# SamShue/EKF_SLAM

Hardware: AMD Instinct MI355X
Metric: EKF update-steps/sec at N landmarks; HBM GB/s on (I−KH)P vs roofline (higher is better)
Workload: dtype f64

## Files before the change

ekf_slam_amd/_lib.py:

```python
import ctypes
import os
import subprocess

_HERE = os.path.dirname(os.path.abspath(__file__))
LIB_PATH = os.environ.get("EKF_LIB_PATH") or os.path.join(_HERE, "libekfslam.so")

EKF_OK = 0
EKF_ERR_INVALID_ARG, EKF_ERR_NO_DEVICE, EKF_ERR_HIP, EKF_ERR_CAPACITY = 1, 2, 3, 4
EKF_ERR_INDEX, EKF_ERR_LOOKUP, EKF_ERR_STATE, EKF_ERR_COMM = 5, 6, 7, 8
EKF_MODE_KNOWN, EKF_MODE_UC = 0, 1
EKF_COMM_ID_BYTES = 128
EKF_MERGE_BATCH_MAX = 32
EKF_STORE_F64, EKF_STORE_F32 = 0, 1
EKF_ARITH_F64, EKF_ARITH_F32, EKF_ARITH_SPLIT3 = 0, 1, 2
(EKF_KERNEL_DOWNDATE, EKF_KERNEL_GATHER, EKF_KERNEL_PREDICT, EKF_KERNEL_ASSOCIATE, EKF_KERNEL_APPEND,
 EKF_KERNEL_ROWPANEL, EKF_KERNEL_EXCHANGE, EKF_KERNEL_COMPACT, EKF_KERNEL_COUNT) = range(9)

_d = ctypes.c_double
_dp = ctypes.POINTER(ctypes.c_double)
_i32 = ctypes.c_int32
_i64 = ctypes.c_int64
_vp = ctypes.c_void_p


class EkfConfig(ctypes.Structure):
    _fields_ = [("C", _d), ("Rc", _d * 2), ("s_cost", _d), ("s_thresh", _d), ("w_pos", _d),
                ("capacity_landmarks", _i64), ("mode", _i32), ("storage", _i32), ("device", _i32),
                ("tile", _i32), ("rank", _i32), ("world", _i32), ("batch", _i32), ("async_flush", _i32), ("device_assoc", _i32),
                ("pass_direction", _i32), ("force_sharded", _i32), ("pass_arith", _i32), ("reserved", _i32 * 2)]


class EkfLinearObs(ctypes.Structure):
    _fields_ = [("z", _d * 2), ("R", _d * 4), ("Hr", _d * 6), ("lm", _i64 * 2), ("Hl", (_d * 4) * 2), ("gate", _d),
                ("wrap_deg", _i32 * 2), ("rows", _i32)]


class EkfLinearResult(ctypes.Structure):
    _fields_ = [("nu", _d * 2), ("S", _d * 4), ("d2", _d), ("outcome", _i32)]


EKF_LINEAR_IRREGULAR, EKF_LINEAR_APPLIED, EKF_LINEAR_GATED = 0, 1, 2


class EkfModelObs(ctypes.Structure):
    _fields_ = [("model", _i32), ("reserved", _i32), ("z", _d * 2), ("R", _d * 4), ("lm", _i64 * 2), ("anchor", _d * 2), ("gate", _d)]


EKF_MODEL_RANGE_BEARING, EKF_MODEL_RANGE, EKF_MODEL_BEARING, EKF_MODEL_RELATIVE_XY, EKF_MODEL_LANDMARK_RANGE = 1, 2, 3, 4, 5
EKF_MODEL_ROWS = {1: 2, 2: 1, 3: 1, 4: 2, 5: 1}

EKF_APPEND_MODEL_MAX = 32

# ... 120 lines not shown
```

ekf_slam_amd/csrc/abi.hip:

```cpp
#include "host/handle.h"
#include "host/invalidate.h"
#include "host/exchange.h"
#include "host/passes.h"
#include "host/steps.h"
#include "host/assoc.h"
#include "host/measure.h"
#include "host/edits.h"
#include "host/linear.h"
#include "host/model.h"
#include "host/append_model.h"
#include "host/associate_model.h"
#include "host/state.h"
#include "host/lifecycle.h"

extern "C" {
int32_t ekf_abi_version(void) { return EKF_ABI_VERSION; }

const char *ekf_status_string(int32_t s) {
    switch (s) {
        case EKF_OK: return "ok";
        case EKF_ERR_INVALID_ARG: return "invalid argument";
        case EKF_ERR_NO_DEVICE: return "no HIP device";
        case EKF_ERR_HIP: return "HIP runtime error";
        case EKF_ERR_CAPACITY: return "landmark capacity exhausted";
// ... 35 lines not shown
    HIPCHK(h, hipStreamSynchronize(h->stream));
    h->stream = hip_stream ? (hipStream_t)hip_stream : h->own_stream;
    return EKF_OK;
}

int32_t ekf_sync(ekf_handle *h) {
    if (!h) return EKF_ERR_INVALID_ARG;
    TRY(enter(h));
    HIPCHK(h, hipStreamSynchronize(h->stream));
    if (h->flush_stream) HIPCHK(h, hipStreamSynchronize(h->flush_stream));
    return EKF_OK;
}

int32_t ekf_flush(ekf_handle *h) {
    if (!h) return EKF_ERR_INVALID_ARG;
    REQUIRE(h, !h->pending, EKF_ERR_STATE, "flush: a sharded correction is between begin and finish");
    int32_t rc = use_device(h);
    if (!rc) rc = settle(h);
    return rc ? rc : flush_pending(h);
}

int32_t ekf_pending(ekf_handle *h, int32_t *npending) {
    if (!h || !npending) return EKF_ERR_INVALID_ARG;
    *npending = h->npend;
    return EKF_OK;
}

int32_t ekf_set_params(ekf_handle *h, double C, const double Rc[2], double s_cost, double s_thresh, double w_pos) {
    if (!h || !Rc) return fail(h, EKF_ERR_INVALID_ARG, "set_params: null argument");
    h->cfg.C = C; h->cfg.Rc[0] = Rc[0]; h->cfg.Rc[1] = Rc[1];
    h->cfg.s_cost = s_cost; h->cfg.s_thresh = s_thresh; h->cfg.w_pos = w_pos;
    return EKF_OK;
}

int32_t ekf_predict(ekf_handle *h, const double u[2]) {
    if (!h || !u) return fail(h, EKF_ERR_INVALID_ARG, "predict: null argument");
    int32_t rc = use_device(h);
    return rc ? rc : do_predict(h, u);
}

int32_t ekf_motion_model(const double *x, int64_t n, const double u[2], double *x_new, double *F) {
    if (!x || !u || !x_new || n < 3) return EKF_ERR_INVALID_ARG;
    const double th = x[2];
    for (int64_t i = 0; i < n; ++i) x_new[i] = x[i];
    x_new[0] = x[0] + u[0] * ekfm::cosd(th + u[1]);
    x_new[1] = x[1] + u[0] * ekfm::sind(th + u[1]);
    x_new[2] = th + u[1];
    if (F) {
        for (int64_t i = 0; i < n * n; ++i) F[i] = 0.0;
        for (int64_t i = 0; i < n; ++i) F[i * n + i] = 1.0;
        F[2 * n + 0] = -1 * u[0] * ekfm::sind(th);
        F[2 * n + 1] = u[0] * ekfm::cosd(th);
    }
    return EKF_OK;
}

int32_t ekf_append(ekf_handle *h, const double u[2], const double R[4], const double pos[2], double signature) {
    if (!h || !u || !R || !pos) return fail(h, EKF_ERR_INVALID_ARG, "append: null argument");
    int32_t rc = use_device(h);
    if (!rc) rc = settle(h);
    return rc ? rc : do_append(h, u, R, pos, signature);
}

int32_t ekf_correct(ekf_handle *h, const double z[2], const double R[4], int64_t idx) {
    if (!h || !z || !R) return fail(h, EKF_ERR_INVALID_ARG, "correct: null argument");
    int32_t rc = use_device(h);
    if (!rc) rc = settle(h);
    return rc ? rc : do_correct(h, z, R, idx);
}

int32_t ekf_associate(ekf_handle *h, const double z[3], const double R[4], int32_t *is_new, int64_t *idx,
                      double *pos_cost, double *sig_cost) {
    if (!h || !z || !R || !is_new || !idx) return fail(h, EKF_ERR_INVALID_ARG, "associate: null argument");
    int32_t rc = use_device(h);
    if (!rc) rc = settle(h);
    return rc ? rc : do_associate(h, z, R, is_new, idx, pos_cost, sig_cost);
}

int32_t ekf_hint_next(ekf_handle *h, int64_t idx) {
    if (!h) return EKF_ERR_INVALID_ARG;
    h->hint_idx = (idx >= 0 && idx < h->N) ? idx : -1;
    return EKF_OK;
}

int32_t ekf_num_landmarks(ekf_handle *h, int64_t *N) {
    if (!h || !N) return fail(h, EKF_ERR_INVALID_ARG, "num_landmarks: null argument");
    if (unsettled(h) > 0) TRY(settle(h));
    *N = h->N;
    return EKF_OK;
}

// ... 21 lines not shown
```

ekf_slam_amd/csrc/host/handle.h:

```cpp
#pragma once
#include "../../../include/ekfslam.h"
#include <hip/hip_runtime.h>
#include <dlfcn.h>
#include <cstdio>
#include <cstdlib>
#include <algorithm>
#include <cmath>
#include <cstring>
#include <new>
#include <string>
#include <vector>

#include "../device_math.h"
#include "../flush32_pipe.h"
#include "../kernels.h"
#include "../layout.h"

struct KernelTimer {
    bool enabled = false;
    std::vector<hipEvent_t> ev;
    size_t used = 0;
};

struct ekf_handle {
    ekf_config cfg;
    int64_t N = 0;
    int64_t cap = 0;
    int32_t T = 64;
    int32_t storage = 0;
    int32_t cur = 0;
    DevState st;
    hipStream_t own_stream = nullptr, stream = nullptr;
    double *h_small = nullptr;
    double *d_digest = nullptr;
    bool have_pp = false;
    PredictArgs pp;
    std::vector<double> s_host;
    mutable std::vector<std::pair<double, int64_t>> s_sorted, s_tail;
    mutable bool s_sorted_ok = false;
    static constexpr size_t kSortedTail = 2048;
    hipEvent_t throttle_ev[2] = { nullptr, nullptr };
    bool throttle_set[2] = { false, false };
    int throttle_k = 0, since_mark = 0;
    int32_t batch = 1;
    int32_t npend = 0;
    int32_t pstart = 0;
    bool async_flush = false;
    void *tilebuf[2] = { nullptr, nullptr };
    int32_t base = 0;
    int32_t nfrozen = 0;
    bool inflight = false;
    int64_t inflight_N = 0;
    bool appended_inflight = false;
    const int64_t *inflight_dn = nullptr;
    int flush_cus = 0;
    hipStream_t flush_stream = nullptr;
    hipEvent_t ev_pairs = nullptr, ev_flushed = nullptr, ev_rows = nullptr;
    PassAux aux = { nullptr, 0, nullptr, 0, 0, nullptr, nullptr };
    int grid_cap = 0;
// ... 143 lines not shown
}

struct DevTemp {
    void **p;
    template <typename Tp> explicit DevTemp(Tp **q) : p((void **)q) {}
    ~DevTemp() { if (*p) hipFree(*p); }
};

template <typename Tp>
int32_t stage_alloc(ekf_handle *h, Tp **area, size_t bytes, hipEvent_t *ev) {
    if (!*area) HIPCHK(h, halloc(h, area, bytes ? bytes : 16, hipHostMallocDefault));
    if (!*ev) HIPCHK(h, new_event(h, ev));
    return EKF_OK;
}
int32_t stage_wait(ekf_handle *h, hipEvent_t ev, bool &busy) { if (busy) { HIPCHK(h, hipEventSynchronize(ev)); busy = false; } return EKF_OK; }
int32_t stage_uploaded(ekf_handle *h, hipEvent_t ev, bool &busy) { HIPCHK(h, hipEventRecord(ev, h->stream)); busy = true; return EKF_OK; }

inline int64_t n_mm(const ekf_handle *h) { return 2 * h->N; }
inline bool decided_mode(const ekf_handle *h) { return h->cfg.mode == EKF_MODE_UC && h->cfg.device_assoc == 4; }
inline int64_t unsettled(const ekf_handle *h) { return decided_mode(h) ? (int64_t)(h->lrec_head - h->lrec_tail) : 0; }
inline int64_t n_hi(const ekf_handle *h) { return h->N + unsettled(h); }
inline size_t elt_size(const ekf_handle *h) { return h->storage == EKF_STORE_F64 ? 8 : 4; }

int32_t use_device(ekf_handle *h) {
    HIPCHK(h, hipSetDevice(h->cfg.device));
    return EKF_OK;
}

struct TimedLaunch {
    hipStream_t s;
    KernelTimer *t;
    hipEvent_t stop = nullptr;
    TimedLaunch(ekf_handle *h, int which) : TimedLaunch(h, which, h->stream) {}
    TimedLaunch(ekf_handle *h, int which, hipStream_t on) : s(on), t(&h->timers[which]) {
        if (!t->enabled) { t = nullptr; return; }
        if (t->used + 2 > t->ev.size()) {
            hipEvent_t a, b;
            if (hipEventCreate(&a) != hipSuccess || hipEventCreate(&b) != hipSuccess) { t = nullptr; return; }
            t->ev.push_back(a); t->ev.push_back(b);
        }
        hipEventRecord(t->ev[t->used], s);
        stop = t->ev[t->used + 1];
        t->used += 2;
    }
    ~TimedLaunch() { if (t) hipEventRecord(stop, s); }
};

#define TIMED(h, which, call) do { TimedLaunch tl_((h), (which)); HIPCHK((h), call); } while (0)

// ... 5 lines not shown
```

ekf_slam_amd/csrc/host/lifecycle.h:

```cpp
#pragma once
namespace {
int32_t create_state(ekf_handle *h) {
    const int64_t ldm = h->st.ldm;
    for (int b = 0; b < 2; ++b) {
        HIPCHK(h, dalloc(h, &h->st.x[b], (size_t)(3 + ldm)));
        HIPCHK(h, dalloc(h, &h->st.prr[b], 16));
        HIPCHK(h, dalloc(h, &h->st.strip[b], (size_t)(3 * ldm)));
        HIPCHK(h, dalloc(h, &h->st.diag[b], (size_t)(3 * h->cap)));
    }
    h->st.dcur = 0;
    HIPCHK(h, dalloc(h, &h->st.s, (size_t)h->cap));
    HIPCHK(h, dalloc(h, &h->st.small, 32));
    HIPCHK(h, dalloc(h, &h->d_digest, kDigestDoubles));
    HIPCHK(h, dalloc(h, &h->d_csmall, 16));
    HIPCHK(h, halloc(h, &h->h_small, 32 * sizeof(double), hipHostMallocDefault));
    const double prr0[9] = { 0.1, 0, 0, 0, 0.1, 0, 0, 0, 0.1 };
    HIPCHK(h, hipMemcpy(h->st.prr[0], prr0, sizeof prr0, hipMemcpyHostToDevice));
    h->cur = 0;
    h->N = 0;
    return EKF_OK;
}
}

extern "C" {
int32_t ekf_create(const ekf_config *cfg, ekf_handle **out) {
    if (!cfg || !out) return EKF_ERR_INVALID_ARG;
    *out = nullptr;
    const int32_t T = cfg->tile == 0 ? (cfg->storage == EKF_STORE_F32 ? 256 : 128) : cfg->tile;
    const int32_t world = cfg->world <= 0 ? 1 : cfg->world;
    if (!(T == 16 || T == 32 || T == 64 || T == 128 || (T == 256 && cfg->storage == EKF_STORE_F32))) return EKF_ERR_INVALID_ARG;
    if (cfg->capacity_landmarks < 1 || cfg->rank < 0 || cfg->rank >= world) return EKF_ERR_INVALID_ARG;
    if (cfg->storage != EKF_STORE_F64 && cfg->storage != EKF_STORE_F32) return EKF_ERR_INVALID_ARG;
    if (cfg->mode != EKF_MODE_KNOWN && cfg->mode != EKF_MODE_UC) return EKF_ERR_INVALID_ARG;
    if (cfg->batch < 0 || cfg->batch > 64) return EKF_ERR_INVALID_ARG;
    if (cfg->mode == EKF_MODE_UC && cfg->device_assoc == 4 && (world > 1 || cfg->force_sharded)) return EKF_ERR_INVALID_ARG;
    if (cfg->pass_arith != EKF_ARITH_F64 &&
        !((cfg->pass_arith == EKF_ARITH_F32 || cfg->pass_arith == EKF_ARITH_SPLIT3) && cfg->storage == EKF_STORE_F32 && T == 256))
        return EKF_ERR_INVALID_ARG;
    int ndev = 0;
    if (hipGetDeviceCount(&ndev) != hipSuccess || ndev <= 0 || cfg->device < 0 || cfg->device >= ndev)
        return EKF_ERR_NO_DEVICE;

    ekf_handle *h = new (std::nothrow) ekf_handle();
    if (!h) return EKF_ERR_INVALID_ARG;
    h->cfg = *cfg;
    h->cfg.world = world;
    h->cfg.tile = T;
    h->T = T;
    h->cap = cfg->capacity_landmarks;
    h->storage = cfg->storage;
    *out = h;

    HIPCHK(h, hipSetDevice(cfg->device));
    hipDeviceProp_t prop = {};
    if (cfg->async_flush != 0 || cfg->pass_arith != EKF_ARITH_F64) HIPCHK(h, hipGetDeviceProperties(&prop, cfg->device));
    {
        int lo = 0, hi = 0;
        HIPCHK(h, hipDeviceGetStreamPriorityRange(&lo, &hi));
        HIPCHK(h, hipStreamCreateWithPriority(&h->own_stream, hipStreamNonBlocking, hi));
    }
    h->stream = h->own_stream;
    const int64_t nt_cap = ekf_tiles_for(2 * h->cap, T);
    h->st.ldm = nt_cap * T;
    h->st.tm = ekf_make_tilemap(T, world, cfg->rank);
    h->work_cap = h->st.tm.slots_for_rows(nt_cap);

    TRY(create_state(h));
    TRY(create_passes(h, prop));
    TRY(create_worklists(h));
    TRY(create_assoc(h));
    TRY(create_exchange(h));
    TRY(create_decided(h));
    TRY(create_linear(h));
// ... 58 lines not shown
```

ekf_slam_amd/csrc/host/steps.h:

```cpp
#pragma once
namespace {
int32_t verify_loop(ekf_handle *h, bool block);
void note_append(ekf_handle *h, double signature);

int32_t materialize_predict(ekf_handle *h) {
    if (!h->have_pp) return EKF_OK;
    h->have_pp = false;
    PredictArgs a = h->pp;
    a.n_mm = 2 * n_hi(h); a.cur = h->cur;
    TIMED(h, EKF_KERNEL_PREDICT, launch_predict(h->st, a, h->storage, h->stream));
    h->cur ^= 1;
    return EKF_OK;
}

int32_t do_predict(ekf_handle *h, const double u[2]) {
    TRY(materialize_predict(h));
    h->pp.u0 = u[0]; h->pp.u1 = u[1]; h->pp.C = h->cfg.C; h->pp.n_mm = 0; h->pp.cur = 0;
    h->have_pp = true;
    static const bool lazy = ekf_tune_int("EKF_LAZY_PREDICT", 1) != 0;
    return lazy ? EKF_OK : materialize_predict(h);
}

int32_t enter(ekf_handle *h) {
    HIPCHK(h, hipSetDevice(h->cfg.device));
    const int32_t rc = verify_loop(h,  true);
    return rc ? rc : materialize_predict(h);
}

int32_t enter_flushed(ekf_handle *h) { TRY(enter(h)); return flush_pending(h); }

int32_t do_append(ekf_handle *h, const double u[2], const double R[4], const double pos[2], double signature,
                  const DevLoopArgs *dl = nullptr) {
    REQUIRE(h, h->N < h->cap, EKF_ERR_CAPACITY, "append: capacity_landmarks exhausted");
    if (h->inflight) h->appended_inflight = true;
    AppendArgs a;
    a.u0 = u[0]; a.u1 = u[1];
    colmajor2(R, a.R00, a.R01, a.R10, a.R11);
    a.pos0 = pos[0]; a.pos1 = pos[1]; a.signature = signature; a.N = h->N; a.cur = h->cur;
    {
// ... 115 lines not shown
            return rc ? rc : finish_step(h);
        }
        int32_t rc = correct_begin(h, z, R, idx);
        if (!rc) rc = run_exchange(h);
        return rc ? rc : correct_finish(h);
    }
    TRY(refresh_work(h));
    CorrectArgs a;
    fill_correct_args(h, a, z, R, idx);
    static const bool fuse_small = ekf_tune_int("EKF_FUSE_SMALL", 1) != 0;
    const bool fused = fuse_small && h->batch == 1 && !h->async_flush && h->npend == 0 && a.n_mm <= gather_fuse_max_rows() &&
                       ekf_tiles_for(a.n_mm, h->T) * h->T <= 256;
    const PredictArgs *fuse = h->have_pp ? &h->pp : nullptr;
    TIMED(h, EKF_KERNEL_GATHER, launch_gather(h->st, a, fuse, h->storage, h->stream, fused));
    h->have_pp = false;
    if (fused) {
        h->cur ^= 1;
        h->st.dcur ^= 1;
        snprintf(h->dd_kernel, sizeof h->dd_kernel, "k_gather<%s,fused downdate>", h->storage == EKF_STORE_F64 ? "double" : "float");
        h->dd_pairs = 1;
        return throttle_step(h);
    }
    return finish_step(h);
}

int32_t do_correct_dev(ekf_handle *h, const double z[2], const double R[4], int64_t idx, const DevLoopArgs &dl) {
    REQUIRE(h, idx >= 0 && idx < h->N, EKF_ERR_INDEX, "correct: landmark index outside the state");
    TRY(refresh_work(h));
    CorrectArgs a;
    fill_correct_args(h, a, z, R, idx);
    if (h->sharded) {
        REQUIRE(h, !h->pending, EKF_ERR_STATE, "correct: an exchange is pending");
        h->slab = slab_for(h, a.n_mm);
        TIMED(h, EKF_KERNEL_ROWPANEL, launch_rowpanel_dev(h->st, a.j, a.n_mm, h->pstart, h->npend, corr_send(h, h->slab), h->storage, h->stream, dl));
        exchange_changed(h);
        h->x_count = h->slab;
        TRY(exchange_bracket(h, 1));
        TRY(gather_sharded(h, a, h->recv, h->slab, 0,  true, &dl));
        return finish_step(h);
    }
    const PredictArgs *fuse = h->have_pp ? &h->pp : nullptr;
    TIMED(h, EKF_KERNEL_GATHER, launch_gather_devloop(h->st, a, fuse, dl, h->storage, h->stream));
    h->have_pp = false;
    return finish_step(h);
}
}
// ... 56 lines not shown
```

ekf_slam_amd/csrc/kernel_args.h:

```cpp
#pragma once
#include <stdint.h>

#include "layout.h"

struct DevState {
    double *x[2];
    double *prr[2];
    double *strip[2];
    void   *tiles;
    double *s;
    double *Gp;
    double *Kp;
    float  *Gp32;
    float  *Kp32;
    int64_t pair_stride;
    int32_t pcap;
    double *small;
    int64_t ldm;
    TileMap tm;
    double *diag[2];
    int32_t dcur;
};

struct PredictArgs {
    double u0, u1, C;
    int64_t n_mm;
// ... 122 lines not shown
```

ekf_slam_amd/csrc/kernels.h:

```cpp
#pragma once
#include <hip/hip_runtime.h>
#include <stdint.h>

#include "device_math.h"
#include "kernel_args.h"
#include "layout.h"

#ifdef EKF_TUNING
#include <stdlib.h>
inline int ekf_tune_int(const char *name, int dflt) { const char *v = getenv(name); return v ? atoi(v) : dflt; }
#else
constexpr int ekf_tune_int(const char *, int dflt) { return dflt; }
#endif

hipError_t launch_predict(const DevState &st, const PredictArgs &a, int storage, hipStream_t s);

hipError_t launch_append(const DevState &st, const AppendArgs &a, int storage, hipStream_t s, const DevLoopArgs *dl = nullptr,
                         const PredictArgs *fused_predict = nullptr);

hipError_t launch_append_model(const DevState &st, const AppendModelArgs &a, int storage, hipStream_t s);

hipError_t launch_gather(const DevState &st, const CorrectArgs &a, const PredictArgs *fused_predict, int storage,
                         hipStream_t s, bool fuse_downdate);
int gather_fuse_max_rows();
hipError_t launch_gather_devloop(const DevState &st, const CorrectArgs &a, const PredictArgs *fused_predict, const DevLoopArgs &dl,
                                 int storage, hipStream_t s);
int64_t gather_workgroups(const DevState &st, int64_t n_mm);
hipError_t launch_gather_decided(const DevState &st, const CorrectArgs &a, const DevLoopArgs &dl, int storage, hipStream_t s);

hipError_t launch_rowpanel(const DevState &st, int64_t j, int64_t n_mm, int pstart, int npend, double *send, int storage,
                           hipStream_t s);
hipError_t launch_rowpanel_dev(const DevState &st, int64_t j, int64_t n_mm, int pstart, int npend, double *send, int storage,
                               hipStream_t s, const DevLoopArgs &dl);
struct RowList { int32_t m; int32_t j[64]; };
hipError_t launch_rowpanel_base(const DevState &st, const int64_t *idx, int m, int64_t n_mm, double *send, int64_t slab,
                                int storage, hipStream_t s);
hipError_t launch_rowpanel_next(const DevState &st, const int64_t *idx, int m, int64_t n_mm, int pstart, int npend, double *send,
                                int64_t slab, int storage, hipStream_t s);
hipError_t launch_gather_sharded(const DevState &st, const CorrectArgs &a, const PredictArgs *fused_predict, const double *recv,
                                 int64_t rank_stride, int64_t offset, bool patched, int storage, hipStream_t s,
                                 const DevLoopArgs *dl = nullptr);

struct AssocDecision {
    int64_t index;
    int32_t is_new;
    int32_t seq;
    double  min_ll;
// ... 84 lines not shown
```

ekf_slam_amd/csrc/kernels.hip:

```cpp
#include "kernels.h"

#include <algorithm>
#include <atomic>
#include <cstdio>
#include <type_traits>

#include "device_math.h"
#include "flush32_mfma.h"
#include "flush32_pipe.h"
#include "flush32_split.h"
#include "flush64_mfma.h"

namespace {

#include "tile_access.h"
#include "lane_ops.h"
#include "predict.h"
#include "assoc_winners.h"
#include "append.h"
#include "append_model.h"
#include "solve_small.h"
#include "rowpanel.h"
#include "pair_column.h"
#include "gather.h"
#include "downdate.h"
#include "associate.h"
#include "state_io.h"
#include "compact.h"
#include "constrain.h"
#include "linear_obs.h"
#include "model_obs.h"
#include "associate_model.h"
#include "merge_pass.h"
#include "nearest.h"

}

#include "launch/dispatch.h"
#include "launch/steps.h"
#include "launch/pass_select.h"
#include "launch/passes.h"
#include "launch/edits.h"
#include "launch/state_io.h"
```

ekf_slam_amd/csrc/launch/steps.h:

```cpp
#pragma once

hipError_t launch_predict(const DevState &st, const PredictArgs &a, int, hipStream_t s) {
    static const int force = ekf_tune_int("EKF_PREDICT_MFMA", -1);
    const bool mfma = force >= 0 ? force != 0 : a.n_mm >= 2048;
    if (mfma) {
        const int64_t nslices = (a.n_mm + 15) / 16;
        int64_t grid = cdiv(nslices > 0 ? nslices : 1, 4);
        if (grid > 1024) grid = 1024;
        hipLaunchKernelGGL(k_predict_mfma, dim3((unsigned)grid), dim3(kBlock), 0, s, st, a);
        return hipGetLastError();
    }
    const int64_t grid = cdiv(a.n_mm > 0 ? a.n_mm : 1, kBlock);
    hipLaunchKernelGGL(k_predict, dim3((unsigned)grid), dim3(kBlock), 0, s, st, a);
    return hipGetLastError();
}

hipError_t launch_append(const DevState &st, const AppendArgs &a, int storage, hipStream_t s, const DevLoopArgs *dlp,
                         const PredictArgs *fused_predict) {
    const int64_t n_mm = 2 * a.N;
    const int64_t grid = cdiv(n_mm > 0 ? n_mm : 1, kBlock);
    const DevLoopArgs dl = dlp ? *dlp : DevLoopArgs{};
    const PredictArgs pa = predict_or_none(fused_predict);
    return with_storage(storage, [&](auto ts) { with_bool(fused_predict != nullptr, [&](auto pred) {
        hipLaunchKernelGGL((k_append<decltype(ts), decltype(pred)::value>), dim3((unsigned)grid), dim3(kBlock), 0, s, st, a, dl, pa);
// ... 19 lines not shown
    typename DevLoopParam<kDev>::type dla{};
    if constexpr (kDev) {
        if (!dl->parts_in || !dl->rec || dl->nblk_in < 1 || a.n_mm < 2) return hipErrorInvalidValue;
        dla = *dl;
    }
    const int64_t grid = gather_workgroups(st, a.n_mm);
    const PredictArgs pa = predict_or_none(fused_predict);
    return with_storage(storage, [&](auto ts) {
        auto launch = [&](auto pred) {
            hipLaunchKernelGGL((k_gather<decltype(ts), kSharded, decltype(pred)::value, kFused, kDev, kDecide>), dim3((unsigned)grid),
                               dim3(kGatherBlock), 0, s, st, a, pv, pa, dla);
        };
        if constexpr (kDecide) launch(std::false_type{});
        else with_bool(fused_predict != nullptr, launch);
    });
}
}

hipError_t launch_gather(const DevState &st, const CorrectArgs &a, const PredictArgs *fused_predict, int storage,
                         hipStream_t s, bool fuse_downdate) {
    if (!fuse_downdate) return gather_form<false, false, false, false>(st, a, fused_predict, PanelView{}, nullptr, storage, s);
    if (a.n_mm > kFuseMaxRows || gather_workgroups(st, a.n_mm) != 1) return hipErrorInvalidValue;
    return gather_form<false, true, false, false>(st, a, fused_predict, PanelView{}, nullptr, storage, s);
}

hipError_t launch_gather_devloop(const DevState &st, const CorrectArgs &a, const PredictArgs *fused_predict, const DevLoopArgs &dl,
                                 int storage, hipStream_t s) {
    return gather_form<false, false, true, false>(st, a, fused_predict, PanelView{}, &dl, storage, s);
}

hipError_t launch_gather_decided(const DevState &st, const CorrectArgs &a, const DevLoopArgs &dl, int storage, hipStream_t s) {
    if (!dl.dn_out || !dl.loc || !dl.abort || (dl.n_known < 0 && !dl.dn_in)) return hipErrorInvalidValue;
    return gather_form<false, false, true, true>(st, a, nullptr, PanelView{}, &dl, storage, s);
}

hipError_t launch_gather_sharded(const DevState &st, const CorrectArgs &a, const PredictArgs *fused_predict, const double *recv,
                                 int64_t rank_stride, int64_t offset, bool patched, int storage, hipStream_t s, const DevLoopArgs *dl) {
    const PanelView pv = { recv, rank_stride, offset,  a.j >> st.tm.shift, patched ? 1 : 0 };
    return dl ? gather_form<true, false, true, false>(st, a, fused_predict, pv, dl, storage, s)
              : gather_form<true, false, false, false>(st, a, fused_predict, pv, nullptr, storage, s);
}

hipError_t launch_rowpanel(const DevState &st, int64_t j, int64_t n_mm, int pstart, int npend, double *send, int storage,
                           hipStream_t s) {
    const int64_t nloc = rowpanel_local_chunks(st.tm, j, n_mm);
    if (nloc == 0) return hipSuccess;
// ... 94 lines not shown
```

include/ekfslam.h:

```cpp
#ifndef EKFSLAM_H
#define EKFSLAM_H

#include <stdint.h>

#ifdef __cplusplus
extern "C" {
#endif

#define EKF_ABI_VERSION 1

enum {
    EKF_OK = 0,
    EKF_ERR_INVALID_ARG = 1,
    EKF_ERR_NO_DEVICE = 2,
    EKF_ERR_HIP = 3,
    EKF_ERR_CAPACITY = 4,
    EKF_ERR_INDEX = 5,
    EKF_ERR_LOOKUP = 6,
    EKF_ERR_STATE = 7,
    EKF_ERR_COMM = 8
};

enum { EKF_MODE_KNOWN = 0,
       EKF_MODE_UC = 1 };
// ... 3 lines not shown
enum { EKF_ARITH_F64 = 0,
       EKF_ARITH_F32 = 1,
       EKF_ARITH_SPLIT3 = 2 };

typedef struct ekf_config {
    double  C;
    double  Rc[2];
    double  s_cost;
    double  s_thresh;
    double  w_pos;
    int64_t capacity_landmarks;
    int32_t mode;
    int32_t storage;
    int32_t device;
    int32_t tile;
    int32_t rank;
    int32_t world;
    int32_t batch;
    int32_t async_flush;
    int32_t device_assoc;
    int32_t pass_direction;
    int32_t force_sharded;
    int32_t pass_arith;
    int32_t reserved[2];
} ekf_config;

typedef struct ekf_handle ekf_handle;

int32_t     ekf_abi_version(void);
const char *ekf_status_string(int32_t status);
int32_t     ekf_config_default(ekf_config *cfg, int32_t mode);

int32_t     ekf_create(const ekf_config *cfg, ekf_handle **out);
int32_t     ekf_destroy(ekf_handle *h);
const char *ekf_last_error(const ekf_handle *h);
int32_t     ekf_set_stream(ekf_handle *h, void *hip_stream);
int32_t     ekf_sync(ekf_handle *h);
int32_t     ekf_flush(ekf_handle *h);
int32_t     ekf_pending(ekf_handle *h, int32_t *npending);
int32_t     ekf_set_params(ekf_handle *h, double C, const double Rc[2], double s_cost, double s_thresh, double w_pos);

int32_t ekf_predict(ekf_handle *h, const double u[2]);

int32_t ekf_motion_model(const double *x, int64_t n, const double u[2], double *x_new, double *F);

int32_t ekf_append(ekf_handle *h, const double u[2], const double R[4], const double pos[2], double signature);

// ... 120 lines not shown
```

Before: 1931.

## Record predict/correct steps into runs executed by one multi-step gather kernel

Adds a recording path that buffers consecutive predict+correct steps into a RunArgs run and executes up to 32 of them in a single k_gather_run launch. Dedicated waves recompute the small pose/covariance solve per step while column lanes apply pending rank-2 patches and keep active landmark columns in LDS. The goal is to cut per-step launch and host round-trip overhead and to reuse loaded column state across steps. In exchange it adds heavy per-block synchronisation, duplicated small solves in every block, and a lot of new code that reaches the existing paths through materialize_run.

Result: no change. 1937, median of 2 (+0.3%).

```diff
diff --git a/ekf_slam_amd/_lib.py b/ekf_slam_amd/_lib.py
--- a/ekf_slam_amd/_lib.py
+++ b/ekf_slam_amd/_lib.py
@@ -27,7 +27,7 @@
     _fields_ = [("C", _d), ("Rc", _d * 2), ("s_cost", _d), ("s_thresh", _d), ("w_pos", _d),
                 ("capacity_landmarks", _i64), ("mode", _i32), ("storage", _i32), ("device", _i32),
                 ("tile", _i32), ("rank", _i32), ("world", _i32), ("batch", _i32), ("async_flush", _i32), ("device_assoc", _i32),
-                ("pass_direction", _i32), ("force_sharded", _i32), ("pass_arith", _i32), ("reserved", _i32 * 2)]
+                ("pass_direction", _i32), ("force_sharded", _i32), ("pass_arith", _i32), ("step_runs", _i32), ("reserved", _i32 * 1)]
 
 
 class EkfLinearObs(ctypes.Structure):
diff --git a/ekf_slam_amd/csrc/abi.hip b/ekf_slam_amd/csrc/abi.hip
--- a/ekf_slam_amd/csrc/abi.hip
+++ b/ekf_slam_amd/csrc/abi.hip
@@ -81,7 +81,7 @@
 
 int32_t ekf_pending(ekf_handle *h, int32_t *npending) {
     if (!h || !npending) return EKF_ERR_INVALID_ARG;
-    *npending = h->npend;
+    *npending = h->npend + h->run.m;
     return EKF_OK;
 }
 
@@ -94,7 +94,7 @@
 
 int32_t ekf_predict(ekf_handle *h, const double u[2]) {
     if (!h || !u) return fail(h, EKF_ERR_INVALID_ARG, "predict: null argument");
-    int32_t rc = use_device(h);
+    int32_t rc = use_device_step(h);
     return rc ? rc : do_predict(h, u);
 }
 
@@ -123,9 +123,9 @@
 
 int32_t ekf_correct(ekf_handle *h, const double z[2], const double R[4], int64_t idx) {
     if (!h || !z || !R) return fail(h, EKF_ERR_INVALID_ARG, "correct: null argument");
-    int32_t rc = use_device(h);
+    int32_t rc = use_device_step(h);
     if (!rc) rc = settle(h);
-    return rc ? rc : do_correct(h, z, R, idx);
+    return rc ? rc : do_correct_recorded(h, z, R, idx);
 }
 
 int32_t ekf_associate(ekf_handle *h, const double z[3], const double R[4], int32_t *is_new, int64_t *idx,
diff --git a/ekf_slam_amd/csrc/gather_run.h b/ekf_slam_amd/csrc/gather_run.h
--- /dev/null
+++ b/ekf_slam_amd/csrc/gather_run.h
@@ -0,0 +1,237 @@
+#pragma once
+#include "run_column.h"
+
+constexpr int kRunCols = 256;
+constexpr int kRunBlock = kRunCols + 3 * 64;
+
+template <typename TS>
+__global__ __launch_bounds__(kRunBlock) void k_gather_run(DevState st, RunArgs ra) {
+    __shared__ double2 tabG[kRunMaxSteps][64], tabK[kRunMaxSteps][64];
+    __shared__ double act[6][64];
+    __shared__ double pss[24];
+    __shared__ SmallSolve sol;
+    __shared__ PredictSmall ps;
+    __shared__ double pose_sh[3];
+    __shared__ double prr_c[9], pose_c[3];
+    const int tid = threadIdx.x;
+    const int role = __builtin_amdgcn_readfirstlane(tid >> 6);
+    const int lane = tid & 63;
+    const int cur = ra.cur;
+    const double *x = cur ? st.x[1] : st.x[0];
+    const double *prr_cur = cur ? st.prr[1] : st.prr[0];
+    double *x_nxt = cur ? st.x[0] : st.x[1];
+    double *strip_nxt = cur ? st.strip[0] : st.strip[1];
+    double *prr_nxt = cur ? st.prr[0] : st.prr[1];
+    const TS *tiles = (const TS *)st.tiles;
+    const int64_t ldm = st.ldm, n_mm = ra.n_mm;
+    const int npend0 = ra.npend, pstart = ra.pstart, m = ra.m;
+    const int64_t ps2 = st.pair_stride / 2;
+    const double2 *Gring = reinterpret_cast<const double2 *>(st.Gp), *Kring = reinterpret_cast<const double2 *>(st.Kp);
+
+    if (role >= 5) {
+        if (role == 5) {
+            if (lane < 9) prr_c[lane] = prr_cur[lane];
+            else if (lane >= 19 && lane < 22) pose_c[lane - 19] = x[lane - 19];
+        }
+        __syncthreads();
+        for (int t = 0; t < m; ++t) {
+            const RunStep &rs = ra.s[t];
+            const int a0 = 2 * rs.slot;
+            const bool pred = rs.has_predict != 0;
+            if (role == 6) {
+                double small_v = 0.0;
+                if (lane < 3) small_v = pose_c[lane];
+                else if (lane < 5) small_v = act[3][a0 + ((lane - 3) & 1)];
+                const double bx = lane_bcast(small_v, 0), by = lane_bcast(small_v, 1), bth = lane_bcast(small_v, 2),
+                             blx = lane_bcast(small_v, 3), bly = lane_bcast(small_v, 4);
+                if (lane == 0) {
+                    double pose[3] = { bx, by, bth };
+                    if (pred) {
+                        const double2 sc2 = sincosd_ni(pose[2] + rs.u1);
+                        const double sn2 = sc2.x, cs2 = sc2.y;
+                        const double p0 = predict_pose_entry(pose, 0, rs.u0, rs.u1, sn2, cs2), p1 = predict_pose_entry(pose, 1, rs.u0, rs.u1, sn2, cs2),
+                                     p2 = predict_pose_entry(pose, 2, rs.u0, rs.u1, sn2, cs2);
+                        pose[0] = p0; pose[1] = p1; pose[2] = p2;
+                    }
+                    const double d0 = blx - pose[0], d1 = bly - pose[1];
+                    const double bearing = bearing_ni(d1, d0, pose[2]);
+                    const double sq = sqrt(d0 * d0 + d1 * d1);
+                    sol.nu[0] = rs.z0 - sq;
+                    sol.nu[1] = rs.z1 - bearing;
+                }
+            } else {
+                double small_v = 0.0;
+                if (lane < 9) small_v = prr_c[lane];
+                else if (lane < 15) small_v = act[(lane - 9) >> 1][a0 + ((lane - 9) & 1)];
+                else if (lane < 19) {
+                    const int q = ((lane - 15) >> 1) + ((lane - 15) & 1);
+                    small_v = q == 0 ? act[4][a0] : q == 1 ? act[5][a0 + 1] : act[4][a0 + 1];
+                }
+                else if (lane < 22) small_v = pose_c[lane - 19];
+                else if (lane < 24) small_v = act[3][a0 + (lane - 22)];
+                if (lane < 24) pss[lane] = small_v;
+                double p[24];
+#pragma unroll
+                for (int i = 0; i < 24; ++i) p[i] = (i >= 15 && i < 19) ? 0.0 : lane_bcast(small_v, i);
+                double fa = 0.0, fb = 0.0;
+                double pose[3] = { p[19], p[20], p[21] };
+                if (pred) {
+                    const double2 sc_l = sincosd_ni((lane & 1) ? pose[2] + rs.u1 : pose[2]);
+                    const double sn = lane_bcast(sc_l.x, 0), cs = lane_bcast(sc_l.y, 0), sn2 = lane_bcast(sc_l.x, 1), cs2 = lane_bcast(sc_l.y, 1);
+                    double W[3];
+                    predict_common(rs.u0, rs.u1, sn, cs, fa, fb, W);
+                    const int ri = lane >= 6 ? 2 : lane >= 3 ? 1 : 0, rj = lane - 3 * ri;
+                    const int ei = ri > rj ? ri : rj, ej = ri > rj ? rj : ri;
+                    const int st_t = (lane - 9) >> 1, st_b = (lane - 9) & 1;
+                    const bool is_prr = lane < 9;
+                    const int g0 = is_prr ? ej : 9 + st_b, g1 = is_prr ? 3 + ej : 11 + st_b, g2 = is_prr ? 6 + ej : 13 + st_b;
+                    const double v0 = lane_gather(small_v, g0 & 63), v1 = lane_gather(small_v, g1 & 63), v2 = lane_gather(small_v, g2 & 63);
+                    const double cj[3] = { v0, v1, v2 };
+                    const double c2[3] = { p[2], p[5], p[8] };
+                    const double wi = EKF_SEL(ei == 0) ? W[0] : (EKF_SEL(ei == 1) ? W[1] : W[2]);
+                    const double wj = EKF_SEL(ej == 0) ? W[0] : (EKF_SEL(ej == 1) ? W[1] : W[2]);
+                    double e_prr, e_q;
+                    predict_prr_entry(ei, ej, cj, c2, fa, fb, wi, wj, rs.C, e_prr, e_q);
+                    double s0 = v0, s1 = v1;
+                    predict_strip(s0, s1, v2, fa, fb);
+                    const double e_strip = EKF_SEL(st_t == 0) ? s0 : (EKF_SEL(st_t == 1) ? s1 : v2);
+                    const double p0 = predict_pose_entry(pose, 0, rs.u0, rs.u1, sn2, cs2), p1 = predict_pose_entry(pose, 1, rs.u0, rs.u1, sn2, cs2),
+                                 p2 = predict_pose_entry(pose, 2, rs.u0, rs.u1, sn2, cs2);
+                    pose[0] = p0; pose[1] = p1; pose[2] = p2;
+                    if (lane < 15) pss[lane] = EKF_SEL(is_prr) ? e_prr : e_strip;
+                    if (lane < 9) ps.Q[lane] = e_q;
+                    if (lane == 0) { ps.fa = fa; ps.fb = fb; }
+                }
+                if (lane < 3) pose_sh[lane] = lane == 0 ? pose[0] : lane == 1 ? pose[1] : pose[2];
+                SmallSolve so;
+                double sq;
+                solve_hs(p[22] - pose[0], p[23] - pose[1], sq, so.Hs);
+                wave_lds_sync();
+                const int ra_ = lane >= 5 ? 1 : 0;
+                double hsel[5];
+#pragma unroll
+                for (int q = 0; q < 5; ++q) hsel[q] = ra_ ? so.Hs[1][q] : so.Hs[0][q];
+                const double e_gs = solve_gs_entry(pss, hsel, lane < 10 ? lane - 5 * ra_ : 0);
+                double GS[2][5];
+#pragma unroll
+                for (int i = 0; i < 10; ++i) GS[i / 5][i % 5] = lane_bcast(e_gs, i);
+                double e_phi;
+                {
+                    const int aa = (lane >> 1) & 1, bb = lane & 1;
+                    double gsel[5], hb[5];
+#pragma unroll
+                    for (int q = 0; q < 5; ++q) { gsel[q] = aa ? GS[1][q] : GS[0][q]; hb[q] = bb ? so.Hs[1][q] : so.Hs[0][q]; }
+                    const double Rab = aa == 0 ? (bb == 0 ? rs.R00 : rs.R01) : (bb == 0 ? rs.R10 : rs.R11);
+                    e_phi = solve_phi_entry(gsel, hb, Rab);
+                }
+                const double phi[4] = { lane_bcast(e_phi, 0), lane_bcast(e_phi, 1), lane_bcast(e_phi, 2), lane_bcast(e_phi, 3) };
+                ekfm::inv2(phi, so.Phi);
+#pragma unroll
+                for (int b = 0; b < 3; ++b) {
+                    so.Gr[0][b] = GS[0][b]; so.Gr[1][b] = GS[1][b];
+#pragma unroll
+                    for (int cc = 0; cc < 2; ++cc) so.Kr[b][cc] = solve_kr_entry(GS[0][b], GS[1][b], so.Phi[cc], so.Phi[2 + cc]);
+                }
+                if (lane == 0) {
+#pragma unroll
+                    for (int i = 0; i < 10; ++i) sol.Hs[i / 5][i % 5] = so.Hs[i / 5][i % 5];
+#pragma unroll
+                    for (int i = 0; i < 4; ++i) sol.Phi[i] = so.Phi[i];
+#pragma unroll
+                    for (int i = 0; i < 6; ++i) { sol.Kr[i / 2][i % 2] = so.Kr[i / 2][i % 2]; sol.Gr[i / 3][i % 3] = so.Gr[i / 3][i % 3]; }
+                }
+            }
+            __syncthreads();
+            if (role == 5) {
+                double nv = 0.0;
+                if (lane < 9) {
+                    const int r = lane / 3, b = lane - 3 * r;
+                    const int rr = r > b ? r : b, bb = r > b ? b : r;
+                    nv = pss[3 * rr + bb] - (sol.Kr[rr][0] * sol.Gr[0][bb] + sol.Kr[rr][1] * sol.Gr[1][bb]);
+                } else if (lane >= 19 && lane < 22) {
+                    const int l = lane - 19;
+                    nv = pose_sh[l] + (sol.Kr[l][0] * sol.nu[0] + sol.Kr[l][1] * sol.nu[1]);
+                }
+                wave_lds_sync();
+                if (lane < 9) prr_c[lane] = nv;
+                else if (lane >= 19 && lane < 22) pose_c[lane - 19] = nv;
+                if (blockIdx.x == 0) {
+                    if (lane >= 32 && lane < 38) { const int q = lane - 32, r = q / 3, b = q - 3 * r; st.small[3 * r + b] = sol.Gr[r][b]; }
+                    else if (lane >= 38 && lane < 44) { const int b = (lane - 38) >> 1, r = (lane - 38) & 1; st.small[6 + 2 * b + r] = sol.Kr[b][r]; }
+                    else if (pred && lane >= 44 && lane < 53) st.small[12 + (lane - 44)] = ps.Q[lane - 44];
+                }
+            }
+            __syncthreads();
+        }
+        if (blockIdx.x == 0 && role == 5) {
+            if (lane < 9) prr_nxt[lane] = prr_c[lane];
+            else if (lane >= 19 && lane < 22) x_nxt[lane - 19] = pose_c[lane - 19];
+        }
+        return;
+    }
+
+    const bool isact = role == 4;
+    int64_t c;
+    bool live;
+    if (isact) {
+        int lj = -1;
+#pragma unroll
+        for (int q = 0; q < kRunMaxSlots; ++q) lj = (lane >> 1) == q ? ra.lm_j[q] : lj;
+        live = (lane >> 1) < ra.nslots && lj >= 0;
+        c = live ? (int64_t)lj + (lane & 1) : 0;
+    } else {
+        c = (int64_t)blockIdx.x * kRunCols + tid;
+        live = c < n_mm;
+    }
+    const int64_t pad_end = st.tm.padded(n_mm);
+    const ColumnOperands o = load_column_operands(st, cur, c, live);
+    RunColumn col = { o.s0, o.s1, o.s2, o.xc, o.dgc, o.dgl };
+    double m0 = 0.0, m1 = 0.0;
+    if (live) run_load_rows<TS>(tiles, st.tm, ra.s[0].j, c, m0, m1);
+    auto publish = [&] { act[0][lane] = col.s0; act[1][lane] = col.s1; act[2][lane] = col.s2; act[3][lane] = col.xc; act[4][lane] = col.dgc; act[5][lane] = col.dgl; };
+    if (isact) {
+        for (int i = 0; i < npend0; ++i) {
+            const int64_t off = (int64_t)ring_slot(pstart, i, st.pcap) * ps2 + c;
+            tabG[i][lane] = live ? Gring[off] : make_double2(0.0, 0.0);
+            tabK[i][lane] = live ? Kring[off] : make_double2(0.0, 0.0);
+        }
+        publish();
+    }
+    __syncthreads();
+
+    for (int t = 0; t < m; ++t) {
+        const RunStep &rs = ra.s[t];
+        const int64_t j = rs.j;
+        const int a0 = 2 * rs.slot;
+        const int np = npend0 + t;
+        const bool rowpart = c <= j, colpart = c >= j + 2;
+        if (live) {
+            const double2 *own_base = (rowpart ? Gring : Kring) + c;
+            auto kj = [&](int i, int b) { return tabK[i][a0 + b]; };
+            auto gj = [&](int i, int b) { return tabG[i][a0 + b]; };
+            if (isact) run_patch_pending(m0, m1, np, rowpart, colpart, [&](int i) { return rowpart ? tabG[i][lane] : tabK[i][lane]; }, kj, gj);
+            else run_patch_pending(m0, m1, np, rowpart, colpart, [&](int i) { return own_base[(int64_t)ring_slot(pstart, i, st.pcap) * ps2]; }, kj, gj);
+        }
+        run_own_block(m0, m1, c, j, col, lane_xor1(col.dgl));
+        double nm0 = 0.0, nm1 = 0.0;
+        if (t + 1 < m && live) run_load_rows<TS>(tiles, st.tm, ra.s[t + 1].j, c, nm0, nm1);
+        __syncthreads();
+
+        double2 gn, kn;
+        run_column_step(col, live, rs.has_predict != 0, ps.fa, ps.fb, sol, m0, m1, gn, kn);
+        run_column_diag(col, kn, gn, make_double2(lane_xor1(gn.x), lane_xor1(gn.y)));
+        if (isact) {
+            tabG[np][lane] = gn;
+            tabK[np][lane] = kn;
+            publish();
+        } else if (c < pad_end)
+            store_pair_column(pair_dest(st, cur, pstart, np, n_mm), c, gn.x, gn.y, kn.x, kn.y);
+        m0 = nm0; m1 = nm1;
+        __syncthreads();
+    }
+    if (!isact && live) {
+        x_nxt[3 + c] = col.xc;
+        strip_nxt[c] = col.s0; strip_nxt[ldm + c] = col.s1; strip_nxt[2 * ldm + c] = col.s2;
+        store_diag_column(buffer_of(st.diag, st.dcur ^ 1), c, col.dgc, col.dgl);
+    }
+}
diff --git a/ekf_slam_amd/csrc/host/handle.h b/ekf_slam_amd/csrc/host/handle.h
--- a/ekf_slam_amd/csrc/host/handle.h
+++ b/ekf_slam_amd/csrc/host/handle.h
@@ -35,6 +35,8 @@
     double *d_digest = nullptr;
     bool have_pp = false;
     PredictArgs pp;
+    bool step_runs = false;
+    RunArgs run = [] { RunArgs r; run_clear(r); return r; }();
     std::vector<double> s_host;
     mutable std::vector<std::pair<double, int64_t>> s_sorted, s_tail;
     mutable bool s_sorted_ok = false;
@@ -224,9 +226,14 @@
 inline int64_t n_hi(const ekf_handle *h) { return h->N + unsettled(h); }
 inline size_t elt_size(const ekf_handle *h) { return h->storage == EKF_STORE_F64 ? 8 : 4; }
 
+int32_t use_device_step(ekf_handle *h) {
+    HIPCHK(h, hipSetDevice(h->cfg.device));
+    return EKF_OK;
+}
+int32_t materialize_run(ekf_handle *h);
 int32_t use_device(ekf_handle *h) {
     HIPCHK(h, hipSetDevice(h->cfg.device));
-    return EKF_OK;
+    return materialize_run(h);
 }
 
 struct TimedLaunch {
diff --git a/ekf_slam_amd/csrc/host/lifecycle.h b/ekf_slam_amd/csrc/host/lifecycle.h
--- a/ekf_slam_amd/csrc/host/lifecycle.h
+++ b/ekf_slam_amd/csrc/host/lifecycle.h
@@ -33,6 +33,7 @@
     if (cfg->storage != EKF_STORE_F64 && cfg->storage != EKF_STORE_F32) return EKF_ERR_INVALID_ARG;
     if (cfg->mode != EKF_MODE_KNOWN && cfg->mode != EKF_MODE_UC) return EKF_ERR_INVALID_ARG;
     if (cfg->batch < 0 || cfg->batch > 64) return EKF_ERR_INVALID_ARG;
+    if (cfg->step_runs != 0 && cfg->step_runs != 1) return EKF_ERR_INVALID_ARG;
     if (cfg->mode == EKF_MODE_UC && cfg->device_assoc == 4 && (world > 1 || cfg->force_sharded)) return EKF_ERR_INVALID_ARG;
     if (cfg->pass_arith != EKF_ARITH_F64 &&
         !((cfg->pass_arith == EKF_ARITH_F32 || cfg->pass_arith == EKF_ARITH_SPLIT3) && cfg->storage == EKF_STORE_F32 && T == 256))
@@ -49,6 +50,7 @@
     h->T = T;
     h->cap = cfg->capacity_landmarks;
     h->storage = cfg->storage;
+    h->step_runs = cfg->step_runs == 0;
     *out = h;
 
     HIPCHK(h, hipSetDevice(cfg->device));
diff --git a/ekf_slam_amd/csrc/host/steps.h b/ekf_slam_amd/csrc/host/steps.h
--- a/ekf_slam_amd/csrc/host/steps.h
+++ b/ekf_slam_amd/csrc/host/steps.h
@@ -4,6 +4,7 @@
 void note_append(ekf_handle *h, double signature);
 
 int32_t materialize_predict(ekf_handle *h) {
+    TRY(materialize_run(h));
     if (!h->have_pp) return EKF_OK;
     h->have_pp = false;
     PredictArgs a = h->pp;
@@ -14,7 +15,7 @@
 }
 
 int32_t do_predict(ekf_handle *h, const double u[2]) {
-    TRY(materialize_predict(h));
+    if (h->have_pp) TRY(materialize_predict(h));
     h->pp.u0 = u[0]; h->pp.u1 = u[1]; h->pp.C = h->cfg.C; h->pp.n_mm = 0; h->pp.cur = 0;
     h->have_pp = true;
     static const bool lazy = ekf_tune_int("EKF_LAZY_PREDICT", 1) != 0;
@@ -176,6 +177,48 @@
         return throttle_step(h);
     }
     return finish_step(h);
+}
+
+bool run_eligible(const ekf_handle *h) {
+    return h->step_runs && !h->sharded && !h->async_flush && !h->inflight && h->batch >= 2 && run_capacity(h->batch, h->npend) > 0;
+}
+
+int32_t materialize_run(ekf_handle *h) {
+    if (h->run.m == 0) return EKF_OK;
+    RunArgs ra = h->run;
+    run_clear(h->run);
+    if (ra.m == 1) {
+        const bool later_pp = h->have_pp;
+        const PredictArgs later = h->pp;
+        const RunStep &s = ra.s[0];
+        h->have_pp = s.has_predict != 0;
+        if (h->have_pp) { h->pp.u0 = s.u0; h->pp.u1 = s.u1; h->pp.C = s.C; h->pp.n_mm = 0; h->pp.cur = 0; }
+        const double z[2] = { s.z0, s.z1 }, R[4] = { s.R00, s.R10, s.R01, s.R11 };
+        const int32_t rc = do_correct(h, z, R, s.j / 2);
+        h->have_pp = later_pp; h->pp = later;
+        return rc;
+    }
+    TRY(refresh_work(h));
+    ra.n_mm = n_mm(h); ra.cur = h->cur; ra.npend = h->npend; ra.pstart = h->pstart;
+    TIMED(h, EKF_KERNEL_GATHER, launch_gather_run(h->st, ra, h->storage, h->stream));
+    h->cur ^= 1;
+    h->st.dcur ^= 1;
+    h->npend += ra.m;
+    h->hint_idx = -1;
+    int32_t rc = (h->npend - h->nfrozen) >= h->batch ? batch_complete(h) : EKF_OK;
+    for (int t = 0; t < ra.m && !rc; ++t) rc = throttle_step(h);
+    return rc;
+}
+
+int32_t do_correct_recorded(ekf_handle *h, const double z[2], const double R[4], int64_t idx) {
+    REQUIRE(h, idx >= 0 && idx < h->N, EKF_ERR_INDEX, "correct: landmark index outside the state");
+    if (run_eligible(h) && h->run.m >= run_capacity(h->batch, h->npend)) TRY(materialize_run(h));
+    if (!run_eligible(h)) { TRY(materialize_run(h)); return do_correct(h, z, R, idx); }
+    const double u[2] = { h->pp.u0, h->pp.u1 };
+    if (!run_add(h->run, run_capacity(h->batch, h->npend), h->have_pp ? u : nullptr, h->pp.C, z, R, idx))
+        return fail(h, EKF_ERR_STATE, "correct: the recorded run took no further step");
+    h->have_pp = false;
+    return h->npend + h->run.m >= h->batch ? materialize_run(h) : EKF_OK;
 }
 
 int32_t do_correct_dev(ekf_handle *h, const double z[2], const double R[4], int64_t idx, const DevLoopArgs &dl) {
diff --git a/ekf_slam_amd/csrc/kernel_args.h b/ekf_slam_amd/csrc/kernel_args.h
--- a/ekf_slam_amd/csrc/kernel_args.h
+++ b/ekf_slam_amd/csrc/kernel_args.h
@@ -2,6 +2,7 @@
 #include <stdint.h>
 
 #include "layout.h"
+#include "run_steps.h"
 
 struct DevState {
     double *x[2];
diff --git a/ekf_slam_amd/csrc/kernels.h b/ekf_slam_amd/csrc/kernels.h
--- a/ekf_slam_amd/csrc/kernels.h
+++ b/ekf_slam_amd/csrc/kernels.h
@@ -23,6 +23,7 @@
 hipError_t launch_gather(const DevState &st, const CorrectArgs &a, const PredictArgs *fused_predict, int storage,
                          hipStream_t s, bool fuse_downdate);
 int gather_fuse_max_rows();
+hipError_t launch_gather_run(const DevState &st, const RunArgs &a, int storage, hipStream_t s);
 hipError_t launch_gather_devloop(const DevState &st, const CorrectArgs &a, const PredictArgs *fused_predict, const DevLoopArgs &dl,
                                  int storage, hipStream_t s);
 int64_t gather_workgroups(const DevState &st, int64_t n_mm);
diff --git a/ekf_slam_amd/csrc/kernels.hip b/ekf_slam_amd/csrc/kernels.hip
--- a/ekf_slam_amd/csrc/kernels.hip
+++ b/ekf_slam_amd/csrc/kernels.hip
@@ -23,6 +23,7 @@
 #include "rowpanel.h"
 #include "pair_column.h"
 #include "gather.h"
+#include "gather_run.h"
 #include "downdate.h"
 #include "associate.h"
 #include "state_io.h"
diff --git a/ekf_slam_amd/csrc/launch/steps.h b/ekf_slam_amd/csrc/launch/steps.h
--- a/ekf_slam_amd/csrc/launch/steps.h
+++ b/ekf_slam_amd/csrc/launch/steps.h
@@ -65,6 +65,20 @@
     if (!fuse_downdate) return gather_form<false, false, false, false>(st, a, fused_predict, PanelView{}, nullptr, storage, s);
     if (a.n_mm > kFuseMaxRows || gather_workgroups(st, a.n_mm) != 1) return hipErrorInvalidValue;
     return gather_form<false, true, false, false>(st, a, fused_predict, PanelView{}, nullptr, storage, s);
+}
+
+hipError_t launch_gather_run(const DevState &st, const RunArgs &a, int storage, hipStream_t s) {
+    if (a.m < 2 || a.npend < 0 || a.npend + a.m > kRunMaxSteps || a.npend + a.m > st.pcap || a.nslots < 1 || a.nslots > kRunMaxSlots ||
+        a.n_mm < 2 || a.n_mm > st.ldm || st.tm.world != 1)
+        return hipErrorInvalidValue;
+    for (int t = 0; t < a.m; ++t) {
+        const RunStep &s = a.s[t];
+        if (s.j < 0 || (s.j & 1) || s.j + 2 > a.n_mm || s.slot < 0 || s.slot >= a.nslots || a.lm_j[s.slot] != s.j) return hipErrorInvalidValue;
+    }
+    const int64_t grid = gather_workgroups(st, a.n_mm);
+    return with_storage(storage, [&](auto ts) {
+        hipLaunchKernelGGL(k_gather_run<decltype(ts)>, dim3((unsigned)grid), dim3(kRunBlock), 0, s, st, a);
+    });
 }
 
 hipError_t launch_gather_devloop(const DevState &st, const CorrectArgs &a, const PredictArgs *fused_predict, const DevLoopArgs &dl,
diff --git a/ekf_slam_amd/csrc/run_column.h b/ekf_slam_amd/csrc/run_column.h
--- /dev/null
+++ b/ekf_slam_amd/csrc/run_column.h
@@ -0,0 +1,78 @@
+#pragma once
+
+struct RunColumn { double s0, s1, s2, xc, dgc, dgl; };
+
+template <typename TS>
+__device__ __forceinline__ void run_load_rows(const TS *tiles, const TileMap &tm, int64_t j, int64_t c, double &m0, double &m1) {
+    if (c <= j) {
+        const int64_t m = tm.T - 1;
+        const TS *tp = tiles + tm.tile_offset(j >> tm.shift, c >> tm.shift) + ((j & m) << tm.shift) + (c & m);
+        m0 = (double)tp[0]; m1 = (double)tp[tm.T];
+    }
+    else if (c >= j + 2) pmm_low_pair<TS>(tiles, tm, c, j, m0, m1);
+    else pmm_low_pair<TS>(tiles, tm, j + 1, j, m0, m1);
+}
+
+__device__ __forceinline__ void run_patch(double &m0, double &m1, bool rowpart, bool colpart, double2 own, double2 kj0, double2 kj1,
+                                          double2 gj0, double2 gj1) {
+    const double2 k0 = rowpart ? kj0 : (colpart ? own : kj1), k1 = colpart ? own : kj1;
+    const double2 g0 = rowpart ? own : gj0, g1 = rowpart ? own : gj1;
+    m0 = rank2_apply(m0, k0, g0);
+    m1 = rank2_apply(m1, k1, g1);
+}
+
+template <typename Own, typename Kj, typename Gj>
+__device__ __forceinline__ void run_patch_pending(double &m0, double &m1, int np, bool rowpart, bool colpart, Own own, Kj kj, Gj gj) {
+    for (int i0 = 0; i0 < np; i0 += 16) {
+        double2 o[16];
+        const bool second = i0 + 8 < np;
+#pragma unroll
+        for (int q = 0; q < 8; ++q) o[q] = own(i0 + q < np ? i0 + q : np - 1);
+        if (second) {
+#pragma unroll
+            for (int q = 8; q < 16; ++q) o[q] = own(i0 + q < np ? i0 + q : np - 1);
+        }
+#pragma unroll
+        for (int g = 0; g < 16; g += 8) {
+            if (g == 0 || second) {
+#pragma unroll
+                for (int q = g; q < g + 8; ++q) {
+                    const int i = i0 + q < np ? i0 + q : np - 1;
+                    double v0 = m0, v1 = m1;
+                    run_patch(v0, v1, rowpart, colpart, o[q], kj(i, 0), kj(i, 1), gj(i, 0), gj(i, 1));
+                    m0 = i0 + q < np ? v0 : m0; m1 = i0 + q < np ? v1 : m1;
+                }
+            }
+        }
+    }
+}
+
+__device__ __forceinline__ void run_own_block(double &m0, double &m1, int64_t c, int64_t j, const RunColumn &col, double dgl_partner) {
+    if (c == j) { m0 = col.dgc; m1 = dgl_partner; }
+    else if (c == j + 1) { m0 = col.dgl; m1 = col.dgc; }
+}
+
+__device__ __forceinline__ void run_column_step(RunColumn &col, bool live, bool has_predict, double fa, double fb, const SmallSolve &sol,
+                                                double m0, double m1, double2 &gn, double2 &kn) {
+    double g0 = 0.0, g1 = 0.0, k0 = 0.0, k1 = 0.0;
+    if (live) {
+        double s0 = col.s0, s1 = col.s1;
+        const double s2 = col.s2;
+        if (has_predict) predict_strip(s0, s1, s2, fa, fb);
+        g0 = sol.Hs[0][0] * s0 + sol.Hs[0][1] * s1 + sol.Hs[0][2] * s2 + sol.Hs[0][3] * m0 + sol.Hs[0][4] * m1;
+        g1 = sol.Hs[1][0] * s0 + sol.Hs[1][1] * s1 + sol.Hs[1][2] * s2 + sol.Hs[1][3] * m0 + sol.Hs[1][4] * m1;
+        k0 = g0 * sol.Phi[0] + g1 * sol.Phi[2];
+        k1 = g0 * sol.Phi[1] + g1 * sol.Phi[3];
+        col.xc = col.xc + (k0 * sol.nu[0] + k1 * sol.nu[1]);
+        col.s0 = s0 - (sol.Kr[0][0] * g0 + sol.Kr[0][1] * g1);
+        col.s1 = s1 - (sol.Kr[1][0] * g0 + sol.Kr[1][1] * g1);
+        col.s2 = s2 - (sol.Kr[2][0] * g0 + sol.Kr[2][1] * g1);
+    }
+    gn = make_double2(g0, g1);
+    kn = make_double2(k0, k1);
+}
+
+__device__ __forceinline__ void run_column_diag(RunColumn &col, double2 kn, double2 gn, double2 gl) {
+    const double ndc = rank2_apply(col.dgc, kn, gn), ndl = rank2_apply(col.dgl, kn, gl);
+    col.dgc = ndc; col.dgl = ndl;
+}
diff --git a/ekf_slam_amd/csrc/run_steps.h b/ekf_slam_amd/csrc/run_steps.h
--- /dev/null
+++ b/ekf_slam_amd/csrc/run_steps.h
@@ -0,0 +1,54 @@
+#pragma once
+#include <stdint.h>
+
+constexpr int kRunMaxSteps = 32;
+constexpr int kRunMaxSlots = 32;
+
+struct RunStep {
+    double u0, u1, C;
+    double z0, z1;
+    double R00, R01, R10, R11;
+    int32_t j;
+    int32_t slot;
+    int32_t has_predict;
+    int32_t pad;
+};
+
+struct RunArgs {
+    int64_t n_mm;
+    int32_t cur;
+    int32_t npend;
+    int32_t pstart;
+    int32_t m;
+    int32_t nslots;
+    int32_t pad;
+    int32_t lm_j[kRunMaxSlots];
+    RunStep s[kRunMaxSteps];
+};
+
+inline void run_clear(RunArgs &r) {
+    r.n_mm = 0; r.cur = 0; r.npend = 0; r.pstart = 0; r.m = 0; r.nslots = 0; r.pad = 0;
+    for (int q = 0; q < kRunMaxSlots; ++q) r.lm_j[q] = -1;
+}
+
+inline int run_capacity(int batch, int npend) {
+    const int cap = (batch < kRunMaxSteps ? batch : kRunMaxSteps) - npend;
+    return cap > 0 ? cap : 0;
+}
+
+inline bool run_add(RunArgs &r, int capacity, const double *u, double C, const double z[2], const double R[4], int64_t idx) {
+    if (r.m >= capacity || r.m >= kRunMaxSteps) return false;
+    const int32_t j = (int32_t)(2 * idx);
+    int slot = 0;
+    while (slot < r.nslots && r.lm_j[slot] != j) ++slot;
+    if (slot == r.nslots) {
+        if (r.nslots >= kRunMaxSlots) return false;
+        r.lm_j[r.nslots++] = j;
+    }
+    RunStep &s = r.s[r.m++];
+    s.u0 = u ? u[0] : 0.0; s.u1 = u ? u[1] : 0.0; s.C = u ? C : 0.0;
+    s.z0 = z[0]; s.z1 = z[1];
+    s.R00 = R[0]; s.R10 = R[1]; s.R01 = R[2]; s.R11 = R[3];
+    s.j = j; s.slot = slot; s.has_predict = u ? 1 : 0; s.pad = 0;
+    return true;
+}
diff --git a/include/ekfslam.h b/include/ekfslam.h
--- a/include/ekfslam.h
+++ b/include/ekfslam.h
@@ -49,7 +49,8 @@
     int32_t pass_direction;
     int32_t force_sharded;
     int32_t pass_arith;
-    int32_t reserved[2];
+    int32_t step_runs;
+    int32_t reserved[1];
 } ekf_config;
 
 typedef struct ekf_handle ekf_handle;
```
